# SysSec-KAIST/LTESniffer

Hardware: AMD Instinct MI355X
Metric: subframes/s (20 MHz, 150 RNTIs) (higher is better)
Workload: dtype f32+int16

## Files before the change

### ltesniffer_amd/csrc/host/lsn_tables.cc

```cpp
#include "lsn_engine.h"
#include "../../../spec/lte_tables.h"
#include "../kernels/lsn_turbo_core.h"
#include <cmath>
#include <cstdio>
#include <stdexcept>

namespace lsn {

void gold_sequence(uint32_t cinit, uint8_t* c, int len)
{
  uint32_t x1 = 1, x2 = cinit & 0x7FFFFFFFu;
  for (int n = 0; n < 1600 + len; n++) {
    if (n >= 1600) c[n - 1600] = (uint8_t)((x1 ^ x2) & 1u);
    x1 = (x1 >> 1) | ((((x1 >> 3) ^ x1) & 1u) << 30);
    x2 = (x2 >> 1) | ((((x2 >> 3) ^ (x2 >> 2) ^ (x2 >> 1) ^ x2) & 1u) << 30);
  }
}

uint32_t symbol_size(uint32_t nprb, int rates)
{
  if (rates != LSN_RATES_3GPP && rates != LSN_RATES_SRSRAN) return 0;
  const bool srs = rates == LSN_RATES_SRSRAN;
  switch (nprb) {
    case 6: return 128;
// ... 176 lines not shown
  for (int k = 0; k < Nsub / 2; k++) { double a = 2.0 * M_PI * k / Nsub; tw[k] = {(float)std::cos(a), (float)(-std::sin(a))}; }
  if (N != Nsub) {
    std::vector<cf32> t3((size_t)N);
    for (int k = 0; k < N; k++) { double a = 2.0 * M_PI * k / N; t3[k] = {(float)std::cos(a), (float)(-std::sin(a))}; }
    cd.twiddle3 = upload(dev_allocs, t3);
  }
  lsn_nco_tables(coarse.data(), fine.data());
  cd.twiddle = upload(dev_allocs, tw); cd.nco_coarse = upload(dev_allocs, coarse); cd.nco_fine = upload(dev_allocs, fine);
  {
    const float s = 0.70710678118654752440f;
    std::vector<cf32> crs((size_t)10 * P * 4 * cd.nref);
    std::vector<uint8_t> c(440);
    const uint32_t nsl = cell.nslot();
    for (uint32_t sf = 0; sf < 10; sf++)
      for (uint32_t p0 = 0; p0 < P; p0 += 2)
        for (int q = 0; q < (p0 == 0 ? 4 : 2); q++) {
          const uint32_t l = p0 == 0 ? (uint32_t)(q >> 1) * nsl + ((q & 1) ? nsl - 3 : 0) : (uint32_t)q * nsl + 1, ns = 2 * sf + (l >= nsl ? 1 : 0), lsl = l % nsl;
          gold_sequence(1024u * (7u * (ns + 1) + lsl + 1) * (2u * id + 1) + 2u * id + (cell.cp ? 0u : 1u), c.data(), 440);
          for (uint32_t m = 0; m < cd.nref; m++) {
            const uint32_t mp = m + 110 - nprb;
            cf32 v{c[2 * mp] ? -s : s, c[2 * mp + 1] ? -s : s};
            for (uint32_t p = p0; p < p0 + 2 && p < P; p++) crs[((sf * P + p) * 4 + q) * cd.nref + m] = v;
          }
        }
    cd.crs = upload(dev_allocs, crs);
  }
  {
    const int nre = (int)cd.nre, n0 = nre / 6;
    std::vector<uint8_t> used0((size_t)n0, 0);
    const int kbar = 6 * (int)(id % (2 * nprb));
    for (int i = 0; i < 4; i++) { int k = (kbar + (i * (int)nprb / 2) * 6) % nre; cd.pcfich_k0[i] = (uint32_t)k; used0[k / 6] = 1; }
    const int ng = (int)((cell.phich_ng_x6 * nprb + 47) / 48);
    std::vector<int> avail;
    for (int i = 0; i < n0; i++) if (!used0[i]) avail.push_back(i);
    const int na = (int)avail.size();
    for (int m = 0; m < ng; m++) for (int i = 0; i < 3; i++) used0[avail[((int)id + m + (i * na) / 3) % na]] = 1;
    std::vector<uint16_t> rk(3 * 800, 0);
    std::vector<uint8_t> rl(3 * 800, 0);
    std::vector<uint16_t> rq(3 * 800, 0xFFFFu);
    auto wof = [&](int l) { return ((cd.reg_w6 >> l) & 1u) ? 6 : 4; };
    for (int cfi = 1; cfi <= 3; cfi++) {
      const int nsym = cfi + (nprb <= 10 ? 1 : 0);
      std::vector<std::pair<uint16_t, uint8_t>> regs;
      for (int k = 0; k < nre; k++)
        for (int l = 0; l < nsym; l++) {
          const int w = wof(l);
          if (k % w || (l == 0 && used0[k / 6])) continue;
          regs.push_back({(uint16_t)k, (uint8_t)l});
        }
      const int M = (int)regs.size(), R = (M + 31) / 32, ND = 32 * R - M;
      std::vector<int> perm;
      for (int j = 0; j < 32; j++) for (int r = 0; r < R; r++) { int idx = r * 32 + lsn_perm_cc[j]; if (idx >= ND) perm.push_back(idx - ND); }
      cd.nof_regs[cfi - 1] = (uint32_t)M; cd.nof_cce[cfi - 1] = (uint32_t)(M / 9);
      for (int mp = 0; mp < M; mp++) {
        const int q = perm[(mp + (int)id) % M];
        if (q < 800) {
          rk[(cfi - 1) * 800 + q] = regs[mp].first; rl[(cfi - 1) * 800 + q] = regs[mp].second;
          const int l = regs[mp].second;
          int nat = regs[mp].first / wof(l);
          for (int j = 0; j < l; j++) nat += nre / wof(j);
          if (nat < 800) rq[(cfi - 1) * 800 + nat] = (uint16_t)q;
        }
      }
    }
    cd.reg_k0 = upload(dev_allocs, rk); cd.reg_l = upload(dev_allocs, rl); cd.reg_q = upload(dev_allocs, rq);
  }
  {
    std::vector<uint8_t> scr((size_t)10 * LSN_LLR_STRIDE), pscr(10 * 32);
    for (uint32_t sf = 0; sf < 10; sf++) {
      gold_sequence(sf * 512u + id, scr.data() + (size_t)sf * LSN_LLR_STRIDE, LSN_LLR_STRIDE);
      gold_sequence((sf + 1) * (2u * id + 1) * 512u + id, pscr.data() + sf * 32, 32);
    }
    cd.pdcch_scr = upload(dev_allocs, scr); cd.pcfich_scr = upload(dev_allocs, pscr);
  }
  {
    float sum = 0.0f;
    for (int i = 0; i < 5; i++) { float d = (float)(i - 2); cd.taps[i] = expf(-(d * d) / 2.0f); }
    for (int i = 0; i < 5; i++) sum = sum + cd.taps[i];
    const float inv = 1.0f / sum;
    for (int i = 0; i < 5; i++) cd.taps[i] = cd.taps[i] * inv;
  }
  {
    search->setCell(cell, cd.nof_cce);
    std::vector<uint32_t> sizes(search->sizes(), search->sizes() + search->nofSizes());
    cd.nsizes = (uint32_t)sizes.size();
    for (size_t i = 0; i < sizes.size(); i++) cd.sizes[i] = sizes[i];
    std::vector<uint16_t> rank((size_t)LSN_MAX_SIZES * 3 * LSN_MAX_DCI_D, 0);
    for (size_t si = 0; si < sizes.size(); si++) {
      const int D = (int)sizes[si] + 16, R = (D + 31) / 32, KP = 32 * R, ND = KP - D;
      int nonnull = 0;
      for (int s = 0; s < 3; s++)
        for (int col = 0; col < 32; col++)
          for (int r = 0; r < R; r++) {
            const int idx = r * 32 + lsn_perm_cc[col];
            if (idx >= ND) rank[si * 3 * LSN_MAX_DCI_D + 3 * (idx - ND) + s] = (uint16_t)nonnull++;
          }
    }
    cd.rankmap = upload(dev_allocs, rank);
    std::vector<uint16_t> cw((size_t)(LSN_MAX_SIZES + 1) * 64, 0);
    auto fill = [&](uint16_t* row, uint32_t n) {
      uint32_t w = 1;
      for (int t = 0; t < 16; t++) { w <<= 1; if (w & 0x10000u) w ^= 0x11021u; }
      for (int i = (int)n - 1; i >= 0; i--) {
        if (i < 64) row[i] = (uint16_t)w;
        w <<= 1; if (w & 0x10000u) w ^= 0x11021u;
      }
    };
    for (uint32_t k = 0; k < cd.nsizes; k++) fill(cw.data() + (size_t)k * 64, cd.sizes[k]);
    fill(cw.data() + (size_t)LSN_MAX_SIZES * 64, 24);
    cd.crc16_w = upload(dev_allocs, cw);
    std::vector<uint16_t> prank(120, 0);
    {
      const int D = 40, R = 2, KP = 64, ND = KP - D;
      int nonnull = 0;
      for (int s = 0; s < 3; s++)
        for (int col = 0; col < 32; col++)
          for (int r = 0; r < R; r++) {
            const int idx = r * 32 + lsn_perm_cc[col];
            if (idx >= ND) prank[3 * (idx - ND) + s] = (uint16_t)nonnull++;
          }
    }
    cd.pbch_rank = upload(dev_allocs, prank);
  }
  {
    std::vector<uint16_t> vm((size_t)3 * 14 * nprb, 0);
    const uint32_t cls_sf[3] = {0, 5, 1};
    for (int cl = 0; cl < 3; cl++)
      for (uint32_t l = 0; l < 14; l++)
        for (uint32_t prb = 0; prb < nprb; prb++) {
          uint16_t m = 0;
          for (uint32_t kk = 0; kk < 12; kk++) if (pdsch_re_usable(cell, cls_sf[cl], l, 12 * prb + kk)) m |= (uint16_t)(1u << kk);
          vm[((size_t)cl * 14 + l) * nprb + prb] = m;
        }
    cd.validmask = upload(dev_allocs, vm);
  }
  {
    std::vector<uint8_t> x1v(LSN_GOLD_LEN);
    std::vector<uint32_t> m2(LSN_GOLD_LEN);
    uint32_t x1 = 1;
    uint32_t st[31];
    for (int i = 0; i < 31; i++) st[i] = 1u << i;
    int head = 0;
    for (int n = 0; n < 1600 + LSN_GOLD_LEN; n++) {
      if (n >= 1600) { x1v[n - 1600] = (uint8_t)(x1 & 1u); m2[n - 1600] = st[head]; }
      x1 = (x1 >> 1) | ((((x1 >> 3) ^ x1) & 1u) << 30);
      const uint32_t nm = st[(head + 3) % 31] ^ st[(head + 2) % 31] ^ st[(head + 1) % 31] ^ st[head];
      st[head] = nm;
      head = (head + 1) % 31;
    }
    cd.gold_x1 = upload(dev_allocs, x1v); cd.gold_x2mask = upload(dev_allocs, m2);
  }
  {
    std::vector<uint32_t> ta(6144), tb(6144);
    uint32_t a = 1, b = 1;
    for (int j = 0; j < 6144; j++) {
      ta[j] = a; tb[j] = b;
      a <<= 1; if (a & 0x1000000u) a ^= 0x1864CFBu;
      b <<= 1; if (b & 0x1000000u) b ^= 0x1800063u;
    }
    cd.crc_tab_a = upload(dev_allocs, ta); cd.crc_tab_b = upload(dev_allocs, tb);
  }
  {
    std::vector<uint32_t> il(turbo_il_offset(0) + 8);
    for (int i = 0; i < LSN_QPP_NSIZES; i++) {
      const int K = lsn_qpp_table[i][0];
      lsn_turbo_il_fill(il.data() + turbo_il_offset(K), K, lsn_qpp_table[i][1], lsn_qpp_table[i][2]);
    }
    cd.turbo_il = upload(dev_allocs, il);
  }
  if (cfg.harq_mode) {
    if (!sh->harq_pool_owner || sh->harq_pool_owner == this) {
      d_harq_pool = dalloc<uint32_t>(dev_allocs, (size_t)HarqDatabase::NENT * HarqDatabase::NPID * 2 * HARQ_SLOT_WORDS);
      sh->harq_pool_owner = this;
      harq_db = HarqDatabase();
      harq_keep.clear();
    }
  }
  h_prune_ring = halloc<uint32_t>(host_allocs, (size_t)PRUNE_RING * LSN_PRUNE_SNAP_WORDS);
  std::memset(h_prune_ring, 0, (size_t)PRUNE_RING * LSN_PRUNE_SNAP_WORDS * sizeof(uint32_t));
  prune_pub.store(0);
  publishPruneSnapshot();
  for (int i = 0; i < nslots; i++) allocChunk(chunks[i]);
  for (int i = 0; i < ndec; i++) allocRunner(runner_c[i]);
  allocRunner(runner_s);
  allocRunner(runner_f);
  allocRunner(runner_k);
  d_iq_staging = dalloc<cf32>(dev_allocs, (size_t)STAGING_SLOTS * max_batch * cfg.nof_rx_antennas * cd.sflen);
}

}
```

### ltesniffer_amd/csrc/kernels/lsn_turbo_core.h

```cpp
#pragma once
#include <stdint.h>
#include <type_traits>
#include "lsn_rm.h"
#ifndef LSN_NEG_METRIC
#define LSN_NEG_METRIC (-12000)
#define LSN_EXT_CLIP 2047
#endif

typedef short lsn_s2 __attribute__((ext_vector_type(2)));
typedef lsn_s2 s2;

#ifdef LSN_TURBO_RANGE_CHECK
#include <cstdio>
#include <cstdlib>
static inline s2 pk_chk(int x, int y, const char* what)
{
  if (x < -32768 || x > 32767 || y < -32768 || y > 32767) { std::fprintf(stderr, "int16 range exceeded in %s: %d %d\n", what, x, y); std::abort(); }
  return s2{(short)x, (short)y};
}
static inline s2 pka(s2 a, s2 b) { return pk_chk((int)a.x + (int)b.x, (int)a.y + (int)b.y, "add"); }
static inline s2 pks(s2 a, s2 b) { return pk_chk((int)a.x - (int)b.x, (int)a.y - (int)b.y, "sub"); }
#else
LSN_HD s2 pka(s2 a, s2 b) { return a + b; }
LSN_HD s2 pks(s2 a, s2 b) { return a - b; }
// ... 257 lines not shown
#ifdef __HIP_DEVICE_COMPILE__
#define LSN_LOCAL_ADDR(x) asm volatile("" : "+v"(x))
#else
#define LSN_LOCAL_ADDR(x) (void)(x)
#endif
  const uint32_t bias2 = (uint32_t)m.bias * 0x10001u;
  const int nsb = lsn_turbo_nsb(W);
  s2 a[4], b[4];
  auto a_start = [&]() {
    if (wl == 0) {
      a[0] = s2{0, (short)LSN_NEG_METRIC};
      a[1] = a[2] = a[3] = s2{(short)LSN_NEG_METRIC, (short)LSN_NEG_METRIC};
    } else {
      for (int k = 0; k < 4; k++) a[k] = nii_a[k];
    }
  };
  a_start();
  uint32_t nx[TB_S / 2];
  uint32_t cur[TB_S / 2];
  auto il_load = [&](int sb) {
    const int w0 = lsn_turbo_sb(W, sb).word;
#pragma unroll
    for (int u = 0; u < TB_S / 2; u++)
      nx[u] = (il + (uint32_t)((w0 + u) * P))[wl] + bias2;
  };
  if (IL) il_load(0);
  uint32_t g[TB_S];
  auto build2 = [&](int tb, int u) {
    const int nat0 = (tb + u) * P + wlb, nat1 = nat0 + P;
    if (IL) {
      const int i0 = (int)(cur[u >> 1] & 0xFFFFu), i1 = (int)(cur[u >> 1] >> 16);
      lsn_operands2<20>(m.spp[i0], m.spp[i1], (uint16_t)m.ext[i0], (uint16_t)m.ext[i1], m.spp[nat0], m.spp[nat1], &g[u], &g[u + 1]);
    } else {
      const uint32_t w0 = m.spp[nat0], w1 = m.spp[nat1];
      lsn_operands2<10>(w0, w1, (uint16_t)m.ext[nat0], (uint16_t)m.ext[nat1], w0, w1, &g[u], &g[u + 1]);
    }
  };
  for (int sb = 0; sb + 1 < nsb; sb++) {
    LSN_LOCAL_ADDR(wlb);
    if (sb >= 1) lsn_ckpt_store(m.ckpt, nt, sb - 1, lane, a, m.cw, m.ch);
    const LsnSubBlock s = lsn_turbo_sb(W, sb);
    const int tb = s.start, n = s.len;
    if (IL) {
#pragma unroll
      for (int u = 0; u < TB_S / 2; u++) cur[u] = nx[u];
      il_load(sb + 1);
    }
    if (n == TB_S) {
#pragma unroll
      for (int u = 0; u < TB_S; u += 2) build2(tb, u);
#pragma unroll
      for (int u = 0; u < TB_S; u += 2) {
        lsn_step_fwd_pk<false>(a, pk_s2(g[u]));
        lsn_step_fwd_pk<true>(a, pk_s2(g[u + 1]));
        LSN_FWD_SWEEP_COUNT(2);
      }
    } else {
#pragma unroll
      for (int u = 0; u < TB_S; u += 2)
        if (u < n) build2(tb, u);
#pragma unroll
      for (int u = 0; u < TB_S; u += 2) {
        if (u + 1 < n) {
          lsn_step_fwd_pk<false>(a, pk_s2(g[u]));
          lsn_step_fwd_pk<true>(a, pk_s2(g[u + 1]));
          LSN_FWD_SWEEP_COUNT(2);
        } else if (u < n) {
          lsn_step_fwd_pk<true>(a, pk_s2(g[u]));
          LSN_FWD_SWEEP_COUNT(1);
        }
      }
    }
  }
  if (wl == P - 1) {
    for (int k = 0; k < 4; k++) b[k] = beta_tail[k];
  } else {
    for (int k = 0; k < 4; k++) b[k] = nii_b[k];
  }
  s2 A[TB_S][4];
  auto ext_index = [&](int tb, int u) { return IL ? (int)((u & 1) ? cur[u >> 1] >> 16 : cur[u >> 1] & 0xFFFFu) : (tb + u) * P + wlb; };
  for (int sb = nsb - 1; sb >= 0; sb--) {
    LSN_LOCAL_ADDR(wlb);
    const LsnSubBlock s = lsn_turbo_sb(W, sb);
    const int tb = s.start, n = s.len;
    if (sb + 1 < nsb) {
      if (sb == 0) {
        a_start();
      } else {
        lsn_ckpt_load(m.ckpt, nt, sb - 1, lane, a, m.cw, m.ch);
      }
    }
    if (IL) {
#pragma unroll
      for (int u = 0; u < TB_S / 2; u++) cur[u] = nx[u];
      if (sb > 0) il_load(sb - 1);
    }
    auto subblock = [&](auto fullc) {
      constexpr bool FULL = decltype(fullc)::value;
#pragma unroll
      for (int u = TB_S - 2; u >= 0; u -= 2)
        if (FULL || u < n) build2(tb, u);
      if constexpr (FULL) {
        auto fwd1 = [&](auto uc) {
          constexpr int u = decltype(uc)::value;
          A[u][0] = a[0]; A[u][1] = a[1]; A[u][2] = a[2]; A[u][3] = a[3];
          lsn_cyc_fwd<u % 7>(a, pk_s2(g[u]));
          if (u & 1) {
            const s2 n0 = a[0];
            a[0] = pks_sel<0, 1, 0, 0>(a[0], n0); a[1] = pks_sel<0, 1, 0, 0>(a[1], n0); a[2] = pks_sel<0, 1, 0, 0>(a[2], n0); a[3] = pks_sel<0, 1, 0, 0>(a[3], n0);
          }
        };
#define LSN_IC(n) std::integral_constant<int, n>{}
        fwd1(LSN_IC(0)); fwd1(LSN_IC(1)); fwd1(LSN_IC(2)); fwd1(LSN_IC(3)); fwd1(LSN_IC(4)); fwd1(LSN_IC(5)); fwd1(LSN_IC(6)); fwd1(LSN_IC(7));
        fwd1(LSN_IC(8)); fwd1(LSN_IC(9)); fwd1(LSN_IC(10)); fwd1(LSN_IC(11)); fwd1(LSN_IC(12)); fwd1(LSN_IC(13)); fwd1(LSN_IC(14)); fwd1(LSN_IC(15));
        if (sb == nsb - 1) {
          lsn_cyc_to_c<TB_S % 7>(a);
          const s2 nn = a[0];
          for (int k = 0; k < 4; k++) a_end[k] = pks_sel<0, 1, 0, 0>(a[k], nn);
        }
        lsn_cyc_from_c<TB_S % 7>(b);
        auto bwd2 = [&](auto uc) {
          constexpr int u = decltype(uc)::value;
          s2 M0a, M1a, M0b, M1b;
          lsn_cyc_bwd<u % 7, false>(b, A[u], pk_s2(g[u]), &M0a, &M1a);
          lsn_cyc_bwd<(u - 1) % 7, true>(b, A[u - 1], pk_s2(g[u - 1]), &M0b, &M1b);
          const s2 e = lsn_ext_two(M0a, M1a, pk_s2(g[u]), M0b, M1b, pk_s2(g[u - 1]));
          m.ext[ext_index(tb, u)] = e.x;
          m.ext[ext_index(tb, u - 1)] = e.y;
        };
        bwd2(LSN_IC(15)); bwd2(LSN_IC(13)); bwd2(LSN_IC(11)); bwd2(LSN_IC(9)); bwd2(LSN_IC(7)); bwd2(LSN_IC(5)); bwd2(LSN_IC(3)); bwd2(LSN_IC(1));
#undef LSN_IC
      } else {
#pragma unroll
        for (int u = 0; u < TB_S; u++) {
          if (u < n) {
            A[u][0] = a[0]; A[u][1] = a[1]; A[u][2] = a[2]; A[u][3] = a[3];
            if (u & 1) lsn_step_fwd_pk<true>(a, pk_s2(g[u])); else lsn_step_fwd_pk<false>(a, pk_s2(g[u]));
          }
        }
#pragma unroll
        for (int u = TB_S - 1; u >= 0; u--) {
          if (u < n) {
            s2 M0, M1;
            lsn_step_bwd_pk(b, A[u], pk_s2(g[u]), &M0, &M1);
            m.ext[ext_index(tb, u)] = lsn_ext_one(M0, M1, pk_s2(g[u]));
          }
        }
      }
    };
    if (n == TB_S) subblock(std::true_type{}); else subblock(std::false_type{});
  }
  for (int k = 0; k < 4; k++) b_out[k] = b[k];
}
```

### ltesniffer_amd/csrc/kernels/stage_c.hip

```cpp
#include "lsn_dsp.h"
#include <algorithm>
#include "lsn_rm.h"
#include <type_traits>

#define SQRT1_2F 0.70710678118654752440f
#define SQRT2F 1.41421356237309504880f
#define LLR_Q 180.0f

__global__ __launch_bounds__(64) void k_pdsch_prep(LsnCellDev c, const LsnGrantDev* __restrict__ jobs, uint16_t* __restrict__ prefix)
{
  const LsnGrantDev& g = jobs[blockIdx.x];
  const int lane = threadIdx.x, nprb = (int)c.nof_prb;
  uint16_t* pf = prefix + g.prefix_off;
  const int cls = g.sf_idx == 0 ? 0 : (g.sf_idx == 5 ? 1 : 2);
  uint32_t before = 0;
  for (int l = 0; l < 14; l++) {
    uint32_t run = 0;
    for (int base = 0; base < nprb; base += 64) {
      const int prb = base + lane;
      uint32_t v = 0;
      if (prb < nprb && l >= (int)g.l0 && ((g.prb_mask[l >= (int)c.nslot ? 1 : 0][prb >> 5] >> (prb & 31)) & 1u)) v = (uint32_t)__popc((unsigned)c.validmask[(cls * 14 + l) * nprb + prb]);
      uint32_t inc = v;
#pragma unroll
      for (int off = 1; off < 64; off <<= 1) {
// ... 249 lines not shown
          if (rx == 0) { a = p0; d = p1; br = b.r; bi = b.i; z0r = t0.r; z0i = t0.i; z1r = t1.r; z1i = t1.i; }
          else { a = a + p0; d = d + p1; br = br + b.r; bi = bi + b.i; z0r = z0r + t0.r; z0i = z0i + t0.i; z1r = z1r + t1.r; z1i = z1i + t1.i; }
        }
        a = a + noise; d = d + noise;
        float det = a * d - (br * br + bi * bi);
        cf32 x0, x1;
        x0.r = (d * z0r - (br * z1r - bi * z1i)) / det;
        x0.i = (d * z0i - (br * z1i + bi * z1r)) / det;
        x1.r = (a * z1r - (br * z0r + bi * z0i)) / det;
        x1.i = (a * z1i - (br * z0i - bi * z0r)) / det;
        float w0 = det / d * 4.0f / chan_ref, w1 = det / a * 4.0f / chan_ref;
        if (g.qm[0]) emit(c, (int)g.qm[0], x0, w0, inv_amp, g.cinit[0], idx, out0);
        if (g.qm[1]) emit(c, (int)g.qm[1], x1, w1, inv_amp, g.cinit[1], idx, out1);
      }
      break;
    }
  }
#undef GRID
#undef CE
}
void lsn_launch_pdsch_demod(const LsnCellDev& c, const LsnGrantDev* g, const uint32_t* items, uint32_t nitems, const uint16_t* prefix, const cf32* grid,
                            const cf32* ce, const LsnChest* ch, int16_t* llr, hipStream_t s)
{
  if (nitems) LSN_LAUNCH(k_pdsch_demod, dim3(nitems, 14), dim3(192), 0, s, c, g, items, prefix, grid, ce, ch, llr);
}

#define RM_NT 256
template <bool STAGED>
__device__ __forceinline__ int rm_sum(const int16_t* __restrict__ e, const int16_t* es, int rank, int E, int nn)
{
  int acc = 0;
  for (int k = rank; k < E; k += nn) acc += STAGED ? (int)es[k] : (int)e[k];
  return acc > LSN_LLR_CLIP ? LSN_LLR_CLIP : (acc < -LSN_LLR_CLIP ? -LSN_LLR_CLIP : acc);
}
__global__ __launch_bounds__(RM_NT) void k_rm(const LsnCbDev* __restrict__ cbs, const int16_t* __restrict__ llr, uint32_t* __restrict__ spp_g, uint32_t seg)
{
  extern __shared__ __attribute__((aligned(16))) unsigned char rm_smem[];
  __shared__ LsnRmGeom geom;
  __shared__ LsnRmCol tab[32];
  int16_t* es = (int16_t*)rm_smem;
  const LsnCbDev cb = cbs[blockIdx.x];
  const int tid = threadIdx.x, K = (int)cb.K, F = (int)cb.F, E = (int)cb.E;
  const int P = cb.nwin ? (int)cb.nwin : lsn_turbo_nwin(K), W = K / P;
  const int ND = 32 * ((K + 4 + 31) >> 5) - (K + 4);
  const int16_t* e = llr + cb.e_off;
  const bool staged = (uint32_t)E <= seg;
  if (tid < 64) {
    int c01 = 0, f2 = 0, c2 = 0;
    if (tid < 32) lsn_rm_geom_col(ND, F, tid, &c01, &f2, &c2);
    int i01 = c01, i2 = c2;
#pragma unroll
    for (int off = 1; off < 32; off <<= 1) {
      const int t = __shfl_up(i01, off), u = __shfl_up(i2, off);
      if (tid >= off) { i01 += t; i2 += u; }
    }
    if (tid < 32) { geom.cnt01[tid] = (uint8_t)c01; geom.first2[tid] = (uint8_t)f2; geom.pre01[tid] = i01 - c01; geom.pre2[tid] = i2 - c2; }
    if (tid == 31) { geom.pre01[32] = i01; geom.pre2[32] = i2; }
    __builtin_amdgcn_fence(__ATOMIC_RELEASE, "wavefront"); __builtin_amdgcn_wave_barrier(); __builtin_amdgcn_fence(__ATOMIC_ACQUIRE, "wavefront");
    if (tid == 0) lsn_rm_geom_finish(geom, K, F, (int)cb.rv);
    __builtin_amdgcn_fence(__ATOMIC_RELEASE, "wavefront"); __builtin_amdgcn_wave_barrier(); __builtin_amdgcn_fence(__ATOMIC_ACQUIRE, "wavefront");
    if (tid < 32) tab[tid] = lsn_rm_fast_col(geom, tid);
  }
  if (staged) {
    const uintptr_t a0 = (uintptr_t)e & ~(uintptr_t)15;
    const int skew = (int)(((uintptr_t)e - a0) >> 1);
    const uint4* src = (const uint4*)a0;
    const int end = skew + E, vend = end >> 3;
    for (int v = tid; v <= vend; v += RM_NT) {
      uint4 d = make_uint4(0u, 0u, 0u, 0u);
      if (8 * v < end) d = src[v];
      if (v == vend) {
        const int q = end & 7;
        const uint32_t keep = (q & 1) ? 0x0000FFFFu : 0u;
        switch (q >> 1) { case 0: d.x &= keep; break; case 1: d.y &= keep; break; case 2: d.z &= keep; break; default: d.w &= keep; break; }
      }
      ((uint4*)es)[v] = d;
    }
    es += skew;
  }
  __syncthreads();
  const int nn = geom.nn;
  uint32_t* out = spp_g + cb.spp_off;
  const bool single = staged && E <= nn;
  auto streams = [&](int x, int& v0, int& v1, int& v2) {
    const int y = x + ND;
    int r0, r1;
    lsn_rm_rank01_fast(tab[lsn_rm_col_of(y)], nn, y, &r0, &r1);
    const int r2 = lsn_rm_rank2_fast(tab[lsn_rm_col_of(y - 1)], nn, y - 1);
    if (single) {
      v0 = (int)es[r0 < E ? r0 : E]; v1 = (int)es[r1 < E ? r1 : E]; v2 = (int)es[r2 < E ? r2 : E];
    } else if (staged) {
      v0 = rm_sum<true>(e, es, r0, E, nn); v1 = rm_sum<true>(e, es, r1, E, nn); v2 = rm_sum<true>(e, es, r2, E, nn);
    } else {
      v0 = rm_sum<false>(e, es, r0, E, nn); v1 = rm_sum<false>(e, es, r1, E, nn); v2 = rm_sum<false>(e, es, r2, E, nn);
    }
  };
  int tq = tid / P, tr = tid - tq * P;
  const int dq = RM_NT / P, dr = RM_NT - dq * P;
  for (int t = tid; t < K; t += RM_NT, tq += dq, tr += dr) {
    if (tr >= P) { tr -= P; tq++; }
    const int x = (int)__umul24((uint32_t)tr, (uint32_t)W) + tq;
    int v0, v1, v2;
    streams(x, v0, v1, v2);
    if (x < F) v0 = v1 = -LSN_LLR_CLIP;
    out[t] = ((uint32_t)v0 & 0x3FFu) | (((uint32_t)v1 & 0x3FFu) << 10) | (((uint32_t)v2 & 0x3FFu) << 20);
  }
  if (tid < 4) {
    int v0, v1, v2;
    streams(K + tid, v0, v1, v2);
    out[K + tid] = (uint32_t)v0; out[K + 4 + tid] = (uint32_t)v1; out[K + 8 + tid] = (uint32_t)v2;
  }
}
void lsn_launch_rm(const LsnCbDev* cb, const int16_t* llr, uint32_t* spp, uint32_t ncb, uint32_t emax, hipStream_t s)
{
  static std::atomic<uint64_t> attr_done{0};
  lsn_func_max_lds((const void*)k_rm, 65536, attr_done, "k_rm");
  const uint32_t cap = (65536 - 32) / 2;
  const uint32_t seg = emax < cap ? emax : cap;
  const size_t lds = (((size_t)seg + 16) * 2 + 15) & ~(size_t)15;
  if (ncb) LSN_LAUNCH(k_rm, dim3(ncb), dim3(RM_NT), lds, s, cb, llr, spp, seg);
}

__global__ __launch_bounds__(256) void k_harq_combine(const LsnCbDev* __restrict__ cbs, const uint32_t* __restrict__ keep, uint32_t* pool, uint32_t* scratch, uint32_t copy)
{
  const LsnCbDev cb = cbs[blockIdx.x];
  const uint32_t place = cb.reserved >> 30, off = cb.reserved & 0x3FFFFFFFu;
  const uint32_t* a = (place == 0u ? (const uint32_t*)pool : place == 1u ? (const uint32_t*)scratch : keep) + off;
  const int K = (int)cb.K;
  if (copy) {
    uint32_t* d = pool + cb.spp_off;
    for (int t = threadIdx.x; t < K + 12; t += 256) d[t] = a[t];
    return;
  }
  const uint32_t* c = keep + cb.e_off;
  uint32_t* d = scratch + cb.spp_off;
  auto clip = [](int v) { return v > LSN_LLR_CLIP ? LSN_LLR_CLIP : (v < -LSN_LLR_CLIP ? -LSN_LLR_CLIP : v); };
  for (int t = threadIdx.x; t < K + 12; t += 256) {
    const uint32_t w = c[t], o = a[t];
    if (t < K) {
      const int v0 = clip(((int)(w << 22) >> 22) + ((int)(o << 22) >> 22)), v1 = clip(((int)(w << 12) >> 22) + ((int)(o << 12) >> 22)), v2 = clip(((int)(w << 2) >> 22) + ((int)(o << 2) >> 22));
      d[t] = ((uint32_t)v0 & 0x3FFu) | (((uint32_t)v1 & 0x3FFu) << 10) | (((uint32_t)v2 & 0x3FFu) << 20);
    } else {
      d[t] = (uint32_t)clip((int)w + (int)o);
    }
  }
}
void lsn_launch_harq_combine(const LsnCbDev* cbs, uint32_t ncb, const uint32_t* keep, uint32_t* pool, uint32_t* scratch, bool copy, hipStream_t s)
{
  if (ncb) LSN_LAUNCH(k_harq_combine, dim3(ncb), dim3(256), 0, s, cbs, keep, pool, scratch, copy ? 1u : 0u);
}

#include "lsn_turbo_core.h"

__device__ __forceinline__ uint32_t mulmod24(uint32_t a, uint32_t b, uint32_t poly)
{
  uint32_t r = 0;
#pragma unroll
  for (int i = 23; i >= 0; i--) {
    r <<= 1;
    r ^= (r & 0x1000000u) ? poly : 0u;
    r ^= ((b >> i) & 1u) ? a : 0u;
  }
  return r & 0xFFFFFFu;
}

__device__ __forceinline__ void tb_sync(int nt)
{
  if (nt == 128) { __syncthreads(); return; }
  __builtin_amdgcn_fence(__ATOMIC_RELEASE, "wavefront");
  __builtin_amdgcn_wave_barrier();
  __builtin_amdgcn_fence(__ATOMIC_ACQUIRE, "wavefront");
}

template <bool IL>
__device__ __forceinline__ void map_pass(const TurboLds& m, const uint32_t* il, int nt, int lane, bool active, int K, int P, int W,
                                         s2* nii_a, s2* nii_b, const s2* beta_tail)
{
  s2 a_end[4] = {s2{0, 0}, s2{0, 0}, s2{0, 0}, s2{0, 0}}, b_out[4] = {s2{0, 0}, s2{0, 0}, s2{0, 0}, s2{0, 0}};
  if (active) lsn_map_pass_lane<IL>(m, il, nt, lane, K, P, W, nii_a, nii_b, beta_tail, a_end, b_out);
  tb_sync(nt);
  lsn_ckpt_store(m.ckpt, nt, 0, lane, a_end, m.cw, m.ch);
  lsn_ckpt_store(m.ckpt, nt, 1, lane, b_out, m.cw, m.ch);
  tb_sync(nt);
  const int lm = lane > 0 ? lane - 1 : 0, lq = lane + 1 < nt ? lane + 1 : lane;
  lsn_ckpt_load(m.ckpt, nt, 0, lm, nii_a, m.cw, m.ch);
  lsn_ckpt_load(m.ckpt, nt, 1, lq, nii_b, m.cw, m.ch);
  tb_sync(nt);
}

__device__ __forceinline__ void tail_beta(const int* ts, const int* tp, int* beta)
{
  int b[8], bn[8];
  for (int S = 0; S < 8; S++) b[S] = S == 0 ? 0 : LSN_NEG_METRIC;
  for (int t = 2; t >= 0; t--) {
    for (int S = 0; S < 8; S++) {
      int s1 = (S >> 2) & 1, s2 = (S >> 1) & 1, s3 = S & 1;
      int u = s2 ^ s3, z = s1 ^ s3, Sn = (s1 << 1) | s2;
      bn[S] = b[Sn] + (u ? ts[t] : 0) + (z ? tp[t] : 0);
    }
    for (int S = 0; S < 8; S++) b[S] = bn[S];
  }
  for (int S = 7; S >= 0; S--) beta[S] = b[S] - b[0];
}

__device__ __forceinline__ uint32_t wg_xor(uint32_t v, int16_t* scratch, int tid, int nt)
{
  for (int off = 32; off > 0; off >>= 1) v ^= __shfl_xor(v, off);
  if (nt == 64) return v;
  uint32_t* w = (uint32_t*)scratch;
  __syncthreads();
  if ((tid & 63) == 0) w[tid >> 6] = v;
  __syncthreads();
  v = w[0] ^ w[1];
  __syncthreads();
  return v;
}

#ifndef TB_WAVES_ATTR
#define TB_WAVES_ATTR __attribute__((amdgpu_waves_per_eu(2, 2)))
#endif
template <int NT>
__global__ __launch_bounds__(NT) TB_WAVES_ATTR void k_turbo(const uint32_t* __restrict__ crc_tab_a, const uint32_t* __restrict__ crc_tab_b, const uint32_t* __restrict__ il_tab,
                                              const LsnCbDev* __restrict__ cbs, const uint32_t* __restrict__ spp_g,
                                              uint8_t* __restrict__ payload, LsnCbRes* res, uint32_t kmax, uint32_t nsolo, uint32_t ncb, uint32_t kmax_pair)
{
  extern __shared__ __attribute__((aligned(16))) unsigned char smem[];
#ifdef LSN_TURBO_CYCLES
#define TB_CLOCK() clock64()
#else
#define TB_CLOCK() 0ll
#endif
  const long long tc0 = TB_CLOCK();
  const bool paired = NT == 128 && blockIdx.x >= nsolo;
  const uint32_t wave = (uint32_t)__builtin_amdgcn_readfirstlane((int)(threadIdx.x >> 6));
  const uint32_t cbi = paired ? nsolo + 2u * (blockIdx.x - nsolo) + wave : blockIdx.x;
  if (cbi >= ncb) return;
  if (paired) kmax = kmax_pair;
  const LsnCbDev cb = cbs[cbi];
  if (cb.dep != LSN_CB_NODEP && res[cb.dep].ok == 0u) {
    if ((paired ? (threadIdx.x & 63u) : threadIdx.x) == 0) { LsnCbRes r{}; res[cb.res_idx] = r; }
    return;
  }
  const int lane = paired ? (int)(threadIdx.x & 63u) : (int)threadIdx.x, K = (int)cb.K, F = (int)cb.F;
  const int P = cb.nwin ? (int)cb.nwin : lsn_turbo_nwin(K), W = K / P;
  const uint32_t magicW = ((1u << 20) + (uint32_t)W - 1u) / (uint32_t)W;
  const int nt = (NT == 128 && (paired || P <= 64)) ? 64 : NT;
  if (lane >= nt) return;
  const bool active = lane < P;
  const uint32_t* il = il_tab + cb.il_off;
  TurboLds m;
  const uint32_t kk = kmax + 8u;
  m.spp = (uint32_t*)smem; m.ext = (int16_t*)(m.spp + (paired ? 2u * kk : kmax)); m.ckpt = (uint8_t*)(m.ext + (paired ? 2u * kk : kk));
  m.bias = paired ? (int)(wave * kk) : 0; m.cw = paired ? (int)(wave * (uint32_t)(TB_CKPT_BYTES / 4)) : 0; m.ch = 2 * m.cw;
  int* tail = (int*)(m.ckpt + 2048) + m.cw;
  {
    const uint32_t* src = spp_g + cb.spp_off;
    for (int i = 4 * lane; i < K; i += 4 * nt) *(uint4*)&m.spp[i + m.bias] = *(const uint4*)&src[i];
    for (int i = 8 * lane; i < K; i += 8 * nt) *(uint4*)&m.ext[i + m.bias] = make_uint4(0u, 0u, 0u, 0u);
    if (lane < 12) tail[lane] = (int)src[K + lane];
  }
  tb_sync(nt);
  s2* bt1 = (s2*)(m.ckpt + (paired ? 2u : 1u) * TB_CKPT_BYTES) + (paired ? 8u * wave : 0u);
  s2* bt2 = bt1 + 4;
  if (lane == 0) {
    const int *s4 = tail, *q1 = tail + 4, *q2 = tail + 8;
    int ts1[3] = {s4[0], q2[0], q1[1]}, tp1[3] = {q1[0], s4[1], q2[1]};
    int ts2[3] = {s4[2], q2[2], q1[3]}, tp2[3] = {q1[2], s4[3], q2[3]};
    int b8[8];
    s2 v[4];
    tail_beta(ts1, tp1, b8); lsn_pack_c(b8, v);
    for (int k = 0; k < 4; k++) bt1[k] = v[k];
    tail_beta(ts2, tp2, b8); lsn_pack_c(b8, v);
    for (int k = 0; k < 4; k++) bt2[k] = v[k];
  }
  tb_sync(nt);
  const long long tc1 = TB_CLOCK();
  const uint32_t poly = cb.crc_b ? 0x1800063u : 0x1864CFBu;
  const uint32_t cw = active ? (cb.crc_b ? crc_tab_b : crc_tab_a)[(P - 1 - lane) * W] : 0u;
  s2 na1[4], nb1[4], na2[4], nb2[4];
#pragma unroll
  for (int s = 0; s < 4; s++) { na1[s] = s2{0, 0}; nb1[s] = s2{0, 0}; na2[s] = s2{0, 0}; nb2[s] = s2{0, 0}; }
  int it = 0;
  bool ok = false;
  while (it < (int)cb.max_iter && !ok) {
    map_pass<false>(m, il, nt, lane, active, K, P, W, na1, nb1, bt1);
    map_pass<true>(m, il, nt, lane, active, K, P, W, na2, nb2, bt2);
    it++;
    uint32_t rem = 0;
    if (active) {
      uint32_t q = cw;
      auto step = [&](uint32_t e) {
        uint32_t mk;
        asm("v_bfe_i32 %0, %1, 0, 1" : "=v"(mk) : "v"(e));
        rem ^= mk & q;
        q <<= 1;
        q ^= (q & 0x1000000u) ? poly : 0u;
      };
      int t = W - 1;
      for (int k = W & 7; k > 0; k--, t--) step((uint32_t)m.ext[t * P + lane + m.bias]);
      for (; t >= 7; t -= 8) {
        uint32_t e[8];
#pragma unroll
        for (int k = 0; k < 8; k++) e[k] = (uint32_t)m.ext[(t - k) * P + lane + m.bias];
#pragma unroll
        for (int k = 0; k < 8; k++) step(e[k]);
      }
    }
    ok = wg_xor(rem, (int16_t*)m.ckpt, lane, nt) == 0;
  }
  const int it_run = it;
  const long long tc2 = TB_CLOCK();
  const int nout = (int)cb.out_bytes;
  uint8_t* outp = payload + cb.out_off;
  const int per = (nout + nt - 1) / nt, j0 = lane * per, j1 = (j0 + per < nout) ? j0 + per : nout;
  uint32_t rema = 0;
  for (int j = j0; j < j1; j++) {
    uint32_t byte = 0, e[8];
#pragma unroll
    for (int q = 0; q < 8; q++) e[q] = (uint32_t)m.ext[tr_idx(F + 8 * j + q, W, P, magicW) + m.bias];
#pragma unroll
    for (int q = 0; q < 8; q++) {
      const uint32_t bit = e[q] & 1u;
      byte = (byte << 1) | bit;
      rema = (rema << 1) | bit;
      rema ^= (rema & 0x1000000u) ? 0x1864CFBu : 0u;
    }
    outp[j] = (uint8_t)byte;
  }
  if (j0 < j1) rema = mulmod24(rema, crc_tab_a[8 * (nout - j1)], 0x1864CFBu);
  rema = wg_xor(rema, (int16_t*)m.ckpt, lane, nt);
  if (lane == 0) {
    const long long tc3 = TB_CLOCK();
    LsnCbRes r; r.ok = ok ? 1u : 0u; r.iters = (uint32_t)it; r.rem_a = rema; r.iters_run = (uint32_t)it_run;
    r.cyc_rm = (uint32_t)(tc1 - tc0); r.cyc_map = (uint32_t)(tc2 - tc1); r.cyc_out = (uint32_t)(tc3 - tc2); r.cyc_all = (uint32_t)(tc3 - tc0);
    res[cb.res_idx] = r;
  }
}

size_t lsn_turbo_lds_bytes(uint32_t kmax) { return 6 * (size_t)kmax + 16 + TB_CKPT_BYTES + 64; }
static size_t turbo_lds_bytes_nt(uint32_t kmax, int) { return lsn_turbo_lds_bytes(kmax); }

void lsn_launch_turbo(const LsnCellDev& c, const LsnCbDev* cb, const uint32_t* spp, uint8_t* payload, LsnCbRes* res, uint32_t n128, uint32_t kmax128,
                      uint32_t n64, uint32_t kmax64, hipStream_t s)
{
  lsn_launch_turbo_packed(c, cb, spp, payload, res, n128, kmax128, 0, 0, s);
  static std::atomic<uint64_t> attr64{0};
  lsn_func_max_lds((const void*)k_turbo<64>, (int)turbo_lds_bytes_nt(6144, 64), attr64, "k_turbo<64>");
  auto fix = [](uint32_t k) { return ((k < 512 ? 512u : k) + 7u) & ~7u; };
  if (n64) LSN_LAUNCH(k_turbo<64>, dim3(n64), dim3(64), turbo_lds_bytes_nt(fix(kmax64), 64), s, c.crc_tab_a, c.crc_tab_b, c.turbo_il, cb + n128, spp, payload, res, fix(kmax64), n64, n64, 0u);
}

void lsn_launch_turbo_packed(const LsnCellDev& c, const LsnCbDev* cb, const uint32_t* spp, uint8_t* payload, LsnCbRes* res, uint32_t nsolo, uint32_t kmax_solo,
                             uint32_t npair, uint32_t kmax_pair, hipStream_t s)
{
  static std::atomic<uint64_t> attr128{0};
  lsn_func_max_lds((const void*)k_turbo<128>, (int)turbo_lds_bytes_nt(6144, 128), attr128, "k_turbo<128>");
  auto fix = [](uint32_t k) { return ((k < 512 ? 512u : k) + 7u) & ~7u; };
  if (!nsolo && !npair) return;
  const uint32_t ks = nsolo ? fix(kmax_solo) : 512u, kp = npair ? fix(kmax_pair) : 512u;
  const size_t pair_lds = npair ? 12 * ((size_t)kp + 8) + 2 * TB_CKPT_BYTES + 64 : 0;
  const size_t lds = std::max(nsolo ? turbo_lds_bytes_nt(ks, 128) : (size_t)0, pair_lds);
  LSN_LAUNCH(k_turbo<128>, dim3(nsolo + (npair + 1) / 2), dim3(128), lds, s, c.crc_tab_a, c.crc_tab_b, c.turbo_il, cb, spp, payload, res, ks, nsolo, nsolo + npair, kp);
}
```

Measured before the change: 275,500.

## Rewrite turbo CRC check and output packing with table-weighted windows and fold8

The per-iteration CRC check inside the turbo loop no longer steps an LFSR per bit. It now accumulates bits against a precomputed weight table (the first 24 bits are shifted in directly) and applies one mulmod24 by the lane's column weight. Output byte packing reads each column sequentially with wrap handling in place of a per-bit index division, and reduces the CRC eight bits at a time with a constexpr fold. This removes serial polynomial-reduction dependencies and per-bit index math, but adds table loads and more intricate edge handling, which risks correctness on the remainder paths.

```diff
diff --git a/ltesniffer_amd/csrc/host/lsn_tables.cc b/ltesniffer_amd/csrc/host/lsn_tables.cc
--- a/ltesniffer_amd/csrc/host/lsn_tables.cc
+++ b/ltesniffer_amd/csrc/host/lsn_tables.cc
@@ -352,12 +352,7 @@
   }
   {
     std::vector<uint32_t> ta(6144), tb(6144);
-    uint32_t a = 1, b = 1;
-    for (int j = 0; j < 6144; j++) {
-      ta[j] = a; tb[j] = b;
-      a <<= 1; if (a & 0x1000000u) a ^= 0x1864CFBu;
-      b <<= 1; if (b & 0x1000000u) b ^= 0x1800063u;
-    }
+    lsn_crc24_weights(LSN_CRC24A, ta.data(), 6144); lsn_crc24_weights(LSN_CRC24B, tb.data(), 6144);
     cd.crc_tab_a = upload(dev_allocs, ta); cd.crc_tab_b = upload(dev_allocs, tb);
   }
   {
diff --git a/ltesniffer_amd/csrc/kernels/lsn_turbo_core.h b/ltesniffer_amd/csrc/kernels/lsn_turbo_core.h
--- a/ltesniffer_amd/csrc/kernels/lsn_turbo_core.h
+++ b/ltesniffer_amd/csrc/kernels/lsn_turbo_core.h
@@ -433,3 +433,149 @@
   }
   for (int k = 0; k < 4; k++) b_out[k] = b[k];
 }
+
+constexpr uint32_t LSN_CRC24A = 0x1864CFBu, LSN_CRC24B = 0x1800063u;
+constexpr uint32_t lsn_crc24_xstep(uint32_t a, uint32_t poly) { return ((a << 1) & 0x1000000u) ? ((a << 1) ^ poly) : (a << 1); }
+constexpr uint32_t lsn_crc24_xpow(uint32_t poly, int j)
+{
+  uint32_t a = 1;
+  for (int i = 0; i < j; i++) a = lsn_crc24_xstep(a, poly);
+  return a;
+}
+inline void lsn_crc24_weights(uint32_t poly, uint32_t* dst, int n)
+{
+  uint32_t a = 1;
+  for (int j = 0; j < n; j++) { dst[j] = a; a = lsn_crc24_xstep(a, poly); }
+}
+LSN_HD uint32_t lsn_bit_mask(uint32_t v, int k)
+{
+#ifdef __HIP_DEVICE_COMPILE__
+  return (uint32_t)__builtin_amdgcn_sbfe((int)v, (uint32_t)k, 1u);
+#else
+  return 0u - ((v >> k) & 1u);
+#endif
+}
+LSN_HD uint32_t lsn_bit0_mask(uint32_t e)
+{
+#ifdef __HIP_DEVICE_COMPILE__
+  uint32_t mk;
+  asm("v_bfe_i32 %0, %1, 0, 1" : "=v"(mk) : "v"(e));
+  return mk;
+#else
+  return 0u - (e & 1u);
+#endif
+}
+LSN_HD uint32_t lsn_shift_in(uint32_t acc, uint32_t e)
+{
+#ifdef __HIP_DEVICE_COMPILE__
+  return __builtin_amdgcn_alignbit(e, acc, 1u);
+#else
+  return (e << 31) | (acc >> 1);
+#endif
+}
+LSN_HD uint32_t lsn_xor_and(uint32_t r, uint32_t mk, uint32_t w)
+{
+#ifdef __HIP_DEVICE_COMPILE__
+  return __builtin_amdgcn_bitop3_b32(r, mk, w, 0x78);
+#else
+  return r ^ (mk & w);
+#endif
+}
+LSN_HD uint32_t lsn_mulmod24(uint32_t a, uint32_t b, uint32_t poly)
+{
+  uint32_t r = 0;
+#pragma unroll
+  for (int i = 23; i >= 0; i--) {
+    r <<= 1;
+    r ^= lsn_bit_mask(r, 24) & poly;
+    r ^= lsn_bit_mask(b, i) & a;
+  }
+  return r & 0xFFFFFFu;
+}
+
+LSN_HD uint32_t lsn_crc_window(const int16_t* ext, int col, int P, int W, const uint32_t* wt)
+{
+#ifdef __HIP_DEVICE_COMPILE__
+  int zero = 0;
+  asm volatile("" : "+s"(zero), "+s"(W), "+s"(P), "+v"(col));
+  wt += zero;
+#endif
+  uint32_t e[8], low = 0, rem;
+  const int16_t* p = ext + ((W - 1) * P + col);
+#pragma unroll
+  for (int k = 0; k < 3; k++) {
+#pragma unroll
+    for (int q = 0; q < 8; q++) e[q] = (uint32_t)p[-q * P];
+#pragma unroll
+    for (int q = 0; q < 8; q++) low = lsn_shift_in(low, e[q]);
+    p -= 8 * P;
+  }
+  rem = low >> 8;
+  const int nb = W >> 3, r = W & 7;
+#pragma clang loop vectorize(disable) unroll(disable)
+  for (int k = 3; k < nb; k++) {
+    const uint32_t* w = wt + 8 * k;
+#pragma unroll
+    for (int q = 0; q < 8; q++) e[q] = (uint32_t)p[-q * P];
+#pragma unroll
+    for (int q = 0; q < 8; q++) rem = lsn_xor_and(rem, lsn_bit0_mask(e[q]), w[q]);
+    p -= 8 * P;
+  }
+  if (r) {
+    const uint32_t* w = wt + 8 * nb;
+    p = ext + col;
+    int off = (r - 1) * P;
+#pragma unroll
+    for (int q = 0; q < 7; q++) {
+      e[q] = (uint32_t)p[off];
+      off = off > P ? off - P : 0;
+    }
+#pragma unroll
+    for (int q = 0; q < 7; q++) {
+      const uint32_t wq = w[q];
+      rem = lsn_xor_and(rem, lsn_bit0_mask(e[q]), q < r ? wq : 0u);
+    }
+  }
+  return rem;
+}
+
+LSN_HD uint32_t lsn_crc24a_fold8(uint32_t v)
+{
+  constexpr uint32_t c0 = lsn_crc24_xpow(LSN_CRC24A, 24), c1 = lsn_crc24_xpow(LSN_CRC24A, 25), c2 = lsn_crc24_xpow(LSN_CRC24A, 26), c3 = lsn_crc24_xpow(LSN_CRC24A, 27),
+                     c4 = lsn_crc24_xpow(LSN_CRC24A, 28), c5 = lsn_crc24_xpow(LSN_CRC24A, 29), c6 = lsn_crc24_xpow(LSN_CRC24A, 30), c7 = lsn_crc24_xpow(LSN_CRC24A, 31);
+  uint32_t r = v & 0xFFFFFFu;
+  r ^= lsn_bit_mask(v, 24) & c0; r ^= lsn_bit_mask(v, 25) & c1; r ^= lsn_bit_mask(v, 26) & c2; r ^= lsn_bit_mask(v, 27) & c3;
+  r ^= lsn_bit_mask(v, 28) & c4; r ^= lsn_bit_mask(v, 29) & c5; r ^= lsn_bit_mask(v, 30) & c6; r ^= lsn_bit_mask(v, 31) & c7;
+  return r;
+}
+
+LSN_HD uint32_t lsn_out_run(const int16_t* ext, int bias, int F, int W, int P, uint32_t magicW, int j0, int j1, int per, uint8_t* out)
+{
+  uint32_t r = 0, acc = 0;
+  const int16_t* p = ext;
+  int n = 0;
+  if (j0 < j1) {
+    const int x0 = F + 8 * j0, w0 = (int)(LSN_UMUL24((uint32_t)x0, magicW) >> 20), t0 = x0 - LSN_MUL24(w0, W);
+    p = ext + (LSN_MUL24(t0, P) + w0 + bias);
+    n = W - t0;
+  }
+  const int D = 1 - W * P;
+  for (int b = 0; b < per; b++) {
+    if (b >= 4) r = lsn_crc24a_fold8(r);
+    if (j0 + b < j1) {
+      uint32_t e[8];
+      const int16_t* pw = p + D;
+#pragma unroll
+      for (int q = 0; q < 8; q++) e[q] = (uint32_t)(q < n ? p : pw)[q * P];
+#pragma unroll
+      for (int q = 7; q >= 0; q--) acc = lsn_shift_in(acc, e[q]);
+      const uint32_t byte = acc >> 24;
+      out[j0 + b] = (uint8_t)byte;
+      r = (r << 8) | byte;
+      const bool wrap = n <= 8;
+      p = (wrap ? pw : p) + 8 * P;
+      n += (wrap ? W : 0) - 8;
+    }
+  }
+  return per >= 4 ? lsn_crc24a_fold8(r) : r;
+}
diff --git a/ltesniffer_amd/csrc/kernels/stage_c.hip b/ltesniffer_amd/csrc/kernels/stage_c.hip
--- a/ltesniffer_amd/csrc/kernels/stage_c.hip
+++ b/ltesniffer_amd/csrc/kernels/stage_c.hip
@@ -425,18 +425,6 @@
 
 #include "lsn_turbo_core.h"
 
-__device__ __forceinline__ uint32_t mulmod24(uint32_t a, uint32_t b, uint32_t poly)
-{
-  uint32_t r = 0;
-#pragma unroll
-  for (int i = 23; i >= 0; i--) {
-    r <<= 1;
-    r ^= (r & 0x1000000u) ? poly : 0u;
-    r ^= ((b >> i) & 1u) ? a : 0u;
-  }
-  return r & 0xFFFFFFu;
-}
-
 __device__ __forceinline__ void tb_sync(int nt)
 {
   if (nt == 128) { __syncthreads(); return; }
@@ -548,8 +536,9 @@
   }
   tb_sync(nt);
   const long long tc1 = TB_CLOCK();
-  const uint32_t poly = cb.crc_b ? 0x1800063u : 0x1864CFBu;
-  const uint32_t cw = active ? (cb.crc_b ? crc_tab_b : crc_tab_a)[(P - 1 - lane) * W] : 0u;
+  const uint32_t poly = cb.crc_b ? LSN_CRC24B : LSN_CRC24A;
+  const uint32_t* wt = cb.crc_b ? crc_tab_b : crc_tab_a;
+  const uint32_t cw = active ? wt[(P - 1 - lane) * W] : 0u;
   s2 na1[4], nb1[4], na2[4], nb2[4];
 #pragma unroll
   for (int s = 0; s < 4; s++) { na1[s] = s2{0, 0}; nb1[s] = s2{0, 0}; na2[s] = s2{0, 0}; nb2[s] = s2{0, 0}; }
@@ -561,23 +550,9 @@
     it++;
     uint32_t rem = 0;
     if (active) {
-      uint32_t q = cw;
-      auto step = [&](uint32_t e) {
-        uint32_t mk;
-        asm("v_bfe_i32 %0, %1, 0, 1" : "=v"(mk) : "v"(e));
-        rem ^= mk & q;
-        q <<= 1;
-        q ^= (q & 0x1000000u) ? poly : 0u;
-      };
-      int t = W - 1;
-      for (int k = W & 7; k > 0; k--, t--) step((uint32_t)m.ext[t * P + lane + m.bias]);
-      for (; t >= 7; t -= 8) {
-        uint32_t e[8];
-#pragma unroll
-        for (int k = 0; k < 8; k++) e[k] = (uint32_t)m.ext[(t - k) * P + lane + m.bias];
-#pragma unroll
-        for (int k = 0; k < 8; k++) step(e[k]);
-      }
+      uint32_t cwi = cw;
+      LSN_LOCAL_ADDR(cwi);
+      rem = lsn_mulmod24(lsn_crc_window(m.ext, lane + m.bias, P, W, wt), cwi, poly);
     }
     ok = wg_xor(rem, (int16_t*)m.ckpt, lane, nt) == 0;
   }
@@ -586,21 +561,8 @@
   const int nout = (int)cb.out_bytes;
   uint8_t* outp = payload + cb.out_off;
   const int per = (nout + nt - 1) / nt, j0 = lane * per, j1 = (j0 + per < nout) ? j0 + per : nout;
-  uint32_t rema = 0;
-  for (int j = j0; j < j1; j++) {
-    uint32_t byte = 0, e[8];
-#pragma unroll
-    for (int q = 0; q < 8; q++) e[q] = (uint32_t)m.ext[tr_idx(F + 8 * j + q, W, P, magicW) + m.bias];
-#pragma unroll
-    for (int q = 0; q < 8; q++) {
-      const uint32_t bit = e[q] & 1u;
-      byte = (byte << 1) | bit;
-      rema = (rema << 1) | bit;
-      rema ^= (rema & 0x1000000u) ? 0x1864CFBu : 0u;
-    }
-    outp[j] = (uint8_t)byte;
-  }
-  if (j0 < j1) rema = mulmod24(rema, crc_tab_a[8 * (nout - j1)], 0x1864CFBu);
+  uint32_t rema = lsn_out_run(m.ext, m.bias, F, W, P, magicW, j0, j1, per, outp);
+  if (j0 < j1) rema = lsn_mulmod24(rema, crc_tab_a[8 * (nout - j1)], LSN_CRC24A);
   rema = wg_xor(rema, (int16_t*)m.ckpt, lane, nt);
   if (lane == 0) {
     const long long tc3 = TB_CLOCK();
```

New measurement: 274,600. Within noise of the previous version (-0.3%).
